# niveathika/siddhi

Measured on AMD Instinct MI355X. Metric: events/sec ingested + matches/sec (partitioned pattern, 1–8 GPU); % HBM peak, higher is better.
Workload: dtype f64; 1 GPU; P3; events_per_gpu=100000000, keys_per_gpu=10000000, micro_batch=50000896, call_size=1024, parallelism=key-sharded x1, input=prepartitioned

## Files before the change

### siddhi_amd/csrc/common.h

```cpp
#pragma once
#include <hip/hip_runtime.h>

#include <cstddef>
#include <cstdint>
#include <cstring>
#include <memory>
#include <stdexcept>
#include <string>
#include <type_traits>
#include <utility>
#include <vector>

#include "../../include/siddhi_hip.h"
#include "../../include/siddhi_ir.h"

namespace shd {

struct Error : std::runtime_error {
  int code;
  Error(int c, const std::string& m) : std::runtime_error(m), code(c) {}
};

#define SHD_HIP(call)                                                                  \
  do {                                                                                 \
// ... 145 lines not shown
};

template <class T>
__device__ __forceinline__ T gld(const T* p, int64_t i) {
  typedef __attribute__((address_space(1))) const T* GP;
  return ((GP)p)[i];
}

struct ColSet {
  const void* col[kMaxCols];
  const uint8_t* nul[kMaxCols];
  int32_t type[kMaxCols];
  int32_t ncols;
  const int64_t* ts;
  int64_t n;
};

inline int type_size(int t) {
  switch (t) {
    case SHD_T_STRING: case SHD_T_INT: case SHD_T_FLOAT: return 4;
    case SHD_T_LONG: case SHD_T_DOUBLE: return 8;
    case SHD_T_BOOL: return 1;
  }
  return 8;
}

__host__ __device__ __forceinline__ uint32_t key_bucket_mix(uint32_t k) {
  const uint32_t h = k * 0x9E3779B1u;
  return h ^ (h >> 16);
}

void scan_exclusive_u32(const uint32_t* in, uint32_t* out, int64_t n, uint32_t* total_dev,
                        DevBuf& scratch, hipStream_t s);
void radix_sort_pairs_u32(uint32_t* keys, uint32_t* vals, uint32_t* keys_alt, uint32_t* vals_alt,
                          int64_t n, int bits, DevBuf& scratch, hipStream_t s, bool& result_in_alt);
void radix_sort_pairs_u64(uint64_t* keys, uint32_t* vals, uint64_t* keys_alt, uint32_t* vals_alt,
                          int64_t n, int bits, DevBuf& scratch, hipStream_t s, bool& result_in_alt);
void radix_sort_triples_u32(uint32_t* keys, uint32_t* vals, uint32_t* w, uint32_t* keys_alt, uint32_t* vals_alt,
                            uint32_t* w_alt, int64_t n, int bits, DevBuf& scratch, hipStream_t s, bool& in_alt,
                            bool hashed = false, uint32_t kbase = 0, int shift0 = 0);
void radix_sort_triples_u64(uint64_t* keys, uint32_t* vals, uint32_t* w, uint64_t* keys_alt, uint32_t* vals_alt,
                            uint32_t* w_alt, int64_t n, int bits, DevBuf& scratch, hipStream_t s, bool& in_alt);
const uint32_t* radix_digit_totals(const DevBuf& scratch, int64_t n);
void radix_digit_scan(const uint32_t* hist, int nb, uint32_t* offs, uint32_t* dtot, hipStream_t s);
void reduce_max_u64(const uint64_t* in, int64_t n, uint64_t* out_dev, hipStream_t s);
void fill_iota_u32(uint32_t* out, int64_t n, uint32_t base, hipStream_t s);

}
```

### siddhi_amd/csrc/engine_absent.hip

```cpp
#include "engine.h"
#include "pattern_common.h"

namespace shd {

namespace {

using pat::ExtRows;
using pat::PairCtx;
using pat::BatchRowCtx;

enum : uint8_t { AS_NONE = 0, AS_FIRED = 1, AS_OPEN = 2 };

struct AbsArgs {
  ExtRows x;
  DExprSet es;
  DFilters f1, fx;
  int is_a;
  int sx;
  int64_t T;
  const int64_t* e_off;
  const int64_t* e_now;
  int ne;
};

// ... 437 lines not shown
    }
    const ExtRows x = ext(&b.cs);
    AbsArgs aa{};
    aa.x = x;
    aa.es = dset();
    aa.f1 = dfilters(f1);
    aa.fx = dfilters(fx);
    aa.is_a = isA;
    aa.sx = sx;
    aa.T = T;
    aa.e_off = d_eoff.as<int64_t>();
    aa.e_now = d_enow.as<int64_t>();
    aa.ne = ne;
    const int nblk = grid_for(n_ext, 1, 4096);
    const int64_t tile = ceil_div(ceil_div(n_ext, nblk), kBlock) * kBlock;
    const int ntile = (int)ceil_div(n_ext, tile);
    d_st.reserve(n_ext);
    d_fe.reserve(n_ext * 4);
    d_bcnt.reserve((size_t)2 * ntile * 4);
    d_boff.reserve((size_t)2 * ntile * 4);
    d_blk.reserve((size_t)ntile * sizeof(AbsOut));
    agg.reserve();
    const AbsArgs* d_aa = dev_args(aa);
    if (aa.f1.fp.ok && aa.fx.fp.ok)
      hipLaunchKernelGGL(k_abs_scan<true>, dim3(ntile), dim3(kBlock), 0, s, d_aa, n_ext, d_st.as<uint8_t>(),
                         d_fe.as<int32_t>(), d_bcnt.as<uint32_t>(), d_blk.as<AbsOut>(), tile);
    else
      hipLaunchKernelGGL(k_abs_scan<false>, dim3(ntile), dim3(kBlock), 0, s, d_aa, n_ext, d_st.as<uint8_t>(),
                         d_fe.as<int32_t>(), d_bcnt.as<uint32_t>(), d_blk.as<AbsOut>(), tile);
    SHD_CHECK_LAUNCH();
    hipLaunchKernelGGL(k_abs_fold, dim3(1), dim3(kBlock), 0, s, (const AbsOut*)d_blk.as<AbsOut>(), ntile,
                       &agg.dev()->out);
    SHD_CHECK_LAUNCH();
    scan_exclusive_u32(d_bcnt.as<uint32_t>(), d_boff.as<uint32_t>(), ntile, &agg.dev()->n_fired, d_scan, s);
    scan_exclusive_u32(d_bcnt.as<uint32_t>() + ntile, d_boff.as<uint32_t>() + ntile, ntile, &agg.dev()->n_open, d_scan,
                       s);
    agg.fetch(&AbsentTotals::out, &AbsentTotals::n_open, s);
    SHD_HIP(hipStreamSynchronize(s));
    mark("absent_scan");
    const AbsOut so = agg.host().out;
    const uint32_t n_fired = agg.host().n_fired, n_open = agg.host().n_open;
    if (so.unmono)
      throw NeedNfa("absent pattern engine: event timestamps decrease");
    d_list.reserve((size_t)std::max<uint32_t>(std::max(n_fired, n_open), 1) * 4);
    if (n_fired) {
      hipLaunchKernelGGL(k_abs_list, dim3(ntile), dim3(kBlock), 0, s, (const uint8_t*)d_st.as<uint8_t>(), n_ext, tile,
                         (uint8_t)AS_FIRED, (const uint32_t*)d_boff.as<uint32_t>(), d_list.as<uint32_t>());
      SHD_CHECK_LAUNCH();
      project(x, d_list.as<uint32_t>(), n_fired, d_fe.as<int32_t>(), d_eoff.as<int64_t>(), 0);
    }
    if (n_open) {
      hipLaunchKernelGGL(k_abs_list, dim3(ntile), dim3(kBlock), 0, s, (const uint8_t*)d_st.as<uint8_t>(), n_ext, tile,
                         (uint8_t)AS_OPEN, (const uint32_t*)d_boff.as<uint32_t>() + ntile, d_list.as<uint32_t>());
      SHD_CHECK_LAUNCH();
    }
    carry_rows(x, d_list.as<uint32_t>(), n_open, 0);
    mark("emit_carry");
    SHD_HIP(hipEventRecord(ev1, s));
    stage_end();
    SHD_HIP(hipEventSynchronize(ev1));
    float ms = 0.f;
    SHD_HIP(hipEventElapsedTime(&ms, ev0, ev1));
    seq += n;
    now = now_after;
    counters.events += n;
    counters.partials += (int64_t)so.created;
    counters.partial_scans += (int64_t)so.steps;
    counters.carry = C;
    counters.kernel_ns = (int64_t)(ms * 1e6);
// ... 110 lines not shown
```

### siddhi_amd/csrc/engine_pattern.hip

```cpp
#include <algorithm>
#include <unordered_map>
#include <cmath>
#include <cstdio>
#include <cstdlib>

#include "engine.h"
#include "knobs.h"
#include "pattern_common.h"

namespace shd {

using namespace pat;

namespace {

template <bool FAST>
__global__ __launch_bounds__(kBlock) void k_prepare(const PrepArgs* __restrict__ ap, int64_t n_ext, int64_t stride,
                                                    uint32_t* __restrict__ k32, uint64_t* __restrict__ k64,
                                                    uint32_t* __restrict__ pv, int32_t* __restrict__ tso,
                                                    PrepAgg* __restrict__ blk) {
  const PrepArgs& a = *ap;
  const DExprSet es = a.es;
  PrepAcc acc;
  const int64_t tbase = a.x.batch.ts[0];
// ... 1321 lines not shown
    if (!sts) a.dts[o] = gld(x.batch.ts, br);
    a.dseq[o] = x.seq0 + br;
  }
  a.dkey[o] = kk;
  a.dpend[o] = (uint8_t)((pend_now || (r < x.C && a.pend_old[r])) ? 1 : 0);
}

__global__ __launch_bounds__(kBlock) void k_gather_list(const GatherArgs* __restrict__ ap,
                                                        const uint32_t* __restrict__ olist, int64_t n_open,
                                                        const uint8_t* __restrict__ pst,
                                                        const uint32_t* __restrict__ spv,
                                                        const uint32_t* __restrict__ skey32,
                                                        const uint64_t* __restrict__ skey64) {
  const GatherArgs& a = *ap;
  const ExtRows& x = a.x;
  for (int64_t oi = (int64_t)blockIdx.x * kBlock + threadIdx.x; oi < n_open; oi = n_open) {
    const int64_t p = olist[oi];
    const int64_t o = oi;
    const int64_t r = pv_row(spv[p]);
    const uint64_t kk = !a.partitioned ? 0 : (a.key64 ? skey64[p] : (uint64_t)skey32[p]);
    const bool sts = a.sts32 || a.sts64;
    gather_open_row(a, o, r, kk, sts, (pst[p] & PS_PEND) != 0);
    if (sts) a.dts[o] = a.sts64 ? a.sts64[p] : gld(x.batch.ts, 0) + (int64_t)a.sts32[p];
  }
}

__global__ __launch_bounds__(kBlock) void k_gather_rec(const GatherArgs* __restrict__ ap, int64_t sub, int nsub,
                                                       const uint32_t* __restrict__ rkey,
                                                       const uint32_t* __restrict__ rpv,
                                                       const int32_t* __restrict__ rts,
                                                       const uint32_t* __restrict__ rpos,
                                                       const uint32_t* __restrict__ scnt,
                                                       const uint32_t* __restrict__ soff,
                                                       const uint8_t* __restrict__ pst) {
  const GatherArgs& a = *ap;
  const int lane = threadIdx.x & 63;
  const int st = (int)blockIdx.x * kSubPerTile + (threadIdx.x >> 6);
  const int64_t base = (int64_t)st * sub;
  const uint32_t nrec = scnt[2 * (int64_t)nsub + st];
  const int64_t tbase = gld(a.x.batch.ts, 0);
  const uint64_t below = ((uint64_t)1 << lane) - 1;
  int64_t o0 = soff[st];
  for (uint32_t i0 = 0; i0 < nrec; i0 += 64) {
    const uint32_t i = i0 + lane;
    bool valid = false, pend = false;
    if (i < nrec) {
      const uint32_t rp = rpos[base + i];
      valid = true;
      if (rp & kRecDeferred) {
        const uint8_t ps = pst[rp & ~kRecDeferred];
        valid = (ps & 0x7Fu) == PS_OPEN;
        pend = (ps & PS_PEND) != 0;
      }
    }
    const uint64_t mv = __ballot(valid);
    if (valid) {
      const int64_t o = o0 + __popcll(mv & below);
      gather_open_row(a, o, pv_row(rpv[base + i]), a.partitioned ? (uint64_t)rkey[base + i] : 0, true, pend);
      a.dts[o] = tbase + (int64_t)rts[base + i];
    }
    o0 += __popcll(mv);
  }
}

struct CarryTable {
  DevBuf col[kMaxCols], nul[kMaxCols], ts, key, seq;
  DevBuf pend;
  DevBuf half, bcol[kMaxCols], bnul[kMaxCols], bts, bseq;
  void reserve_b(int64_t n, const std::vector<int>& types) {
    n = std::max<int64_t>(n, 1);
    half.reserve(n);
    for (size_t c = 0; c < types.size(); c++) {
      bcol[c].reserve(n * type_size(types[c]));
      bnul[c].reserve(n);
    }
    bts.reserve(n * 8);
    bseq.reserve(n * 8);
  }
  ColSet colset_b(const std::vector<int>& types, int64_t n) const {
    ColSet cs{};
    cs.ncols = (int)types.size();
    for (size_t c = 0; c < types.size(); c++) {
      cs.col[c] = bcol[c].p;
      cs.nul[c] = bnul[c].as<uint8_t>();
      cs.type[c] = (int32_t)types[c];
    }
    cs.ts = bts.as<int64_t>();
    cs.n = n;
    return cs;
  }
  void reserve(int64_t n, const std::vector<int>& types) {
    for (size_t c = 0; c < types.size(); c++) {
      col[c].reserve(std::max<int64_t>(n, 1) * type_size(types[c]));
      nul[c].reserve(std::max<int64_t>(n, 1));
    }
    ts.reserve(std::max<int64_t>(n, 1) * 8);
    key.reserve(std::max<int64_t>(n, 1) * 8);
    seq.reserve(std::max<int64_t>(n, 1) * 8);
    pend.reserve(std::max<int64_t>(n, 1));
  }
  ColSet colset(const std::vector<int>& types) const {
    ColSet cs{};
    cs.ncols = (int)types.size();
    for (size_t c = 0; c < types.size(); c++) {
      cs.col[c] = col[c].p;
      cs.nul[c] = nul[c].as<uint8_t>();
      cs.type[c] = (int32_t)types[c];
    }
    cs.ts = ts.as<int64_t>();
    return cs;
  }
};

bool expr_reads_only(const Plan& p, int e, int st) {
  for (auto& in : p.exprs[e])
    if ((in.op == SHD_OP_LOAD || in.op == SHD_OP_EVNULL || in.op == SHD_OP_TS) && in.a != st) return false;
  return true;
}

int plain_load_attr(const Plan& p, int e) {
  auto& code = p.exprs[e];
  if (code.size() == 1 && code[0].op == SHD_OP_LOAD) return code[0].c & 0xFFFF;
  return -1;
}

bool find_key_equality(const Plan& p, const std::vector<int>& filters, int& attr_a, int& attr_b, int& type) {
  for (int e : filters) {
    const auto& code = p.exprs[e];
    std::vector<int> st;
    std::vector<std::pair<int, int>> kid(code.size(), {-1, -1});
    bool ok = true;
    for (int i = 0; i < (int)code.size() && ok; i++) {
// ... 632 lines not shown
                           s);
        d_dlist.reserve((size_t)n_ext * 4);
        hipLaunchKernelGGL(k_open_list, dim3(ntile), dim3(kBlock), 0, s, (const uint8_t*)d_pst.as<uint8_t>(),
                           (const uint32_t*)d_boff.as<uint32_t>(), n_ext, tile, d_dlist.as<uint32_t>(),
                           (uint32_t)PS_DEFER, 2);
        SHD_CHECK_LAUNCH();
#define SHD_LAUNCH_RLIST(FAST, TS64)                                                                               \
  hipLaunchKernelGGL((k_resume_list<false, FAST, TS64>), dim3(nlb), dim3(kBlock), 0, s, d_sa, n_ext, tile, ntile,     \
                     skey32, skey64, spv, sts32, sts64, d_match.as<int32_t>(), d_mother.as<int32_t>(),              \
                     d_pst.as<uint8_t>(), d_bcnt.as<uint32_t>(), d_blk.as<ScanOut>(), ntile,                        \
                     (const uint32_t*)d_dlist.as<uint32_t>(), (const uint32_t*)d_ndef, (const uint32_t*)nullptr, 0,  \
                     (int64_t)0, (uint32_t*)nullptr)
        if (fast2) {
          if (ts64) SHD_LAUNCH_RLIST(true, true); else SHD_LAUNCH_RLIST(true, false);
        } else {
          if (ts64) SHD_LAUNCH_RLIST(false, true); else SHD_LAUNCH_RLIST(false, false);
        }
#undef SHD_LAUNCH_RLIST
      } else if (fast2) { SHD_LAUNCH_RESUME2(false, true); }
      else { SHD_LAUNCH_RESUME2(false, false); }
    }
#undef SHD_LAUNCH_RESUME2
#undef SHD_LAUNCH_SKIP
#undef SHD_LAUNCH_RESUME_D
#undef SHD_LAUNCH_RESUME
#undef SHD_LAUNCH_SCAN
    SHD_CHECK_LAUNCH();
    hipLaunchKernelGGL(k_finish_scan, dim3(1), dim3(kBlock), 0, s, (const ScanOut*)d_blk.as<ScanOut>(),
                       rlist ? ntile + nlb : (rmode == 3 && !lockstep ? 3 : 2) * ntile,
                       d_so);
    SHD_CHECK_LAUNCH();
    mark("forward_scan");

    scan_exclusive_u32(d_bcnt.as<uint32_t>(), d_boff.as<uint32_t>(), ntile, &agg.dev()->n_match, d_scan, s);
    if (slists)
      scan_exclusive_u32(d_scnt, d_soff, nsub, &agg.dev()->n_open, d_scan, s);
    else
      scan_exclusive_u32(d_bcnt.as<uint32_t>() + ntile, d_boff.as<uint32_t>() + ntile, ntile, &agg.dev()->n_open,
                         d_scan, s);
    mark("compact");
    agg.fetch(&PatternTotals::scan, &PatternTotals::tail_, s);
    SHD_HIP(hipMemcpyAsync(&h_agg.t_last, b.cs.ts + (n - 1), 8, hipMemcpyDeviceToHost, s));
    SHD_HIP(hipStreamSynchronize(s));
    const ScanOut so = h_agg.scan;
    const uint32_t m = h_agg.n_match;
    const uint32_t n_open = h_agg.n_open;
    if (so.violation)
      throw NeedNfa("pattern engine: event timestamps decrease within a key under `within`");
    if (so.pruned) {
      have_horizon = true;
      horizon = std::max(horizon, t_end);
    }
    fin_sts32 = sts32;
    fin_sts64 = sts64;
    finish(b, x, n_ext, tile, ntile, spv, skey32, skey64, sorted64, keyed, grouped, key64, m, n_open, so, t_end,
           pg.n_cand);
  }

  void finish(const Staged& b, const ExtRows& x, int64_t n_ext, int64_t tile, int ntile, const uint32_t* spv,
              const uint32_t* skey32, const uint64_t* skey64, bool sorted64, bool keyed, bool grouped, bool key64,
              uint32_t m, uint32_t n_open, const ScanOut& so, int64_t t_end, uint64_t n_cand) {
    hipStream_t s = stream;
    const int64_t n = b.n;
    if (m > 0) {
      d_pj.reserve((int64_t)m * 4);
      d_pi.reserve((int64_t)m * 4);
      d_pj_alt.reserve((int64_t)m * 4);
      d_pi_alt.reserve((int64_t)m * 4);
      if (logical == 2) {
        d_se1.reserve((int64_t)m * 4);
        d_sot.reserve((int64_t)m * 4);
      }
      hipLaunchKernelGGL(k_emit_pairs, dim3(ntile), dim3(kBlock), 0, s, (const uint8_t*)d_pst.as<uint8_t>(),
                         (const uint32_t*)d_boff.as<uint32_t>(), (const int32_t*)d_match.as<int32_t>(), spv, n_ext,
                         tile, logical, (const int32_t*)d_mother.as<int32_t>(), d_pj.as<uint32_t>(),
                         d_pi.as<uint32_t>(), d_se1.as<uint32_t>(), d_sot.as<int32_t>());
      SHD_CHECK_LAUNCH();
      int bits = 0;
      while (bits < 32 && ((uint64_t)n_ext >> bits)) bits++;
      if (logical) bits++;
      bool in_alt = false;
      radix_sort_pairs_u32(d_pj.as<uint32_t>(), d_pi.as<uint32_t>(), d_pj_alt.as<uint32_t>(),
                           d_pi_alt.as<uint32_t>(), m, bits, d_sort, s, in_alt);
      const uint32_t* pj = in_alt ? d_pj_alt.as<uint32_t>() : d_pj.as<uint32_t>();
      const uint32_t* pi = in_alt ? d_pi_alt.as<uint32_t>() : d_pi.as<uint32_t>();
      if (!gmembers.empty()) {
        group_emit(b, x, pj, pi, m);
        mark("order_project");
      } else {
        out.ensure(m, s);
        ProjArgs pr{};
        pr.x = x;
        pr.es = dset();
        pr.nout = (int)outs.size();
        pr.fast = 1;
        for (size_t c = 0; c < outs.size(); c++) {
          pr.outs[c] = dexpr(outs[c]);
          if (!fast_atom(outs[c], pr.oat[c])) pr.fast = 0;
        }
        pr.multi = (sA == sB);
        pr.logical = logical;
        pr.s_first = s_first;
        pr.s_second = s_second;
        pr.se1 = d_se1.as<uint32_t>();
        pr.sot = d_sot.as<int32_t>();
        pr.chunk0 = chunk_seq;
        pr.row0 = out.count;
        hipLaunchKernelGGL(k_project, dim3(grid_cover(m)), dim3(kBlock), 0, s, dev_args(pr), pj, pi, (int64_t)m,
                           out.d_chunk(), out.d_type(), out.d_ts(), out.d_vals(), out.d_nulls(), out.d_seq(),
                           out.d_sidx());
        SHD_CHECK_LAUNCH();
        out.count += m;
        if (sA != sB && !logical) chunk_seq += m;
        mark("order_project");
      }
    }

    int nxt = cur ^ 1;
    carry[nxt].reserve(n_open, typesA);
    if (n_open > 0) {
      GatherArgs ga{};
      ga.x = x;
      ga.ncols = (int)typesA.size();
      ga.partitioned = keyed;
      ga.key64 = sorted64;
      for (size_t c = 0; c < typesA.size(); c++) {
        ga.types[c] = (int32_t)typesA[c];
        ga.dcol[c] = carry[nxt].col[c].p;
        ga.dnul[c] = carry[nxt].nul[c].as<uint8_t>();
      }
      ga.dts = carry[nxt].ts.as<int64_t>();
      ga.dkey = carry[nxt].key.as<uint64_t>();
      ga.dseq = carry[nxt].seq.as<int64_t>();
      carry[cur].pend.reserve(std::max<int64_t>(C, 1));
      ga.dpend = carry[nxt].pend.as<uint8_t>();
      ga.pend_old = carry[cur].pend.as<uint8_t>();
      if (logical == 2) {
        carry[nxt].reserve_b(n_open, typesB);
        ga.and_mode = 1;
        ga.match_row = d_match.as<int32_t>();
        ga.dhalf = carry[nxt].half.as<uint8_t>();
        ga.ncolsB = (int)typesB.size();
        for (size_t c = 0; c < typesB.size(); c++) {
          ga.typesB[c] = (int32_t)typesB[c];
          ga.dcolB[c] = carry[nxt].bcol[c].p;
          ga.dnulB[c] = carry[nxt].bnul[c].as<uint8_t>();
        }
        ga.dtsB = carry[nxt].bts.as<int64_t>();
        ga.dseqB = carry[nxt].bseq.as<int64_t>();
      }
      if (keyed && !grouped) {
        ga.key64 = key64;
        skey32 = d_k32.as<uint32_t>();
        skey64 = d_k64.as<uint64_t>();
      }
      if (logical != 2) {
        ga.amask = carry_mask;
        if (grouped) {
          ga.sts32 = fin_sts32;
          ga.sts64 = fin_sts64;
          ga.key_attr = (partitioned && !sorted64 && key_col[0] >= 0 &&
                         (key_type[0] == SHD_T_STRING || key_type[0] == SHD_T_INT)) ? key_col[0] : -1;
        } else {
          ga.key_attr = -1;
        }
        if (fin_rec.on) {
          hipLaunchKernelGGL(k_gather_rec, dim3(ntile), dim3(kBlock), 0, s, dev_args(ga), fin_rec.sub, fin_rec.nsub,
                             (const uint32_t*)fin_rec.key, (const uint32_t*)fin_rec.pv, (const int32_t*)fin_rec.ts,
                             (const uint32_t*)fin_rec.pos,
                             (const uint32_t*)(d_bcnt.as<uint32_t>() + 3 * ntile),
                             (const uint32_t*)(d_boff.as<uint32_t>() + 3 * ntile),
                             (const uint8_t*)d_pst.as<uint8_t>());
        } else {
          d_olist.reserve((size_t)n_open * 4);
          hipLaunchKernelGGL(k_open_list, dim3(ntile), dim3(kBlock), 0, s, (const uint8_t*)d_pst.as<uint8_t>(),
                             (const uint32_t*)d_boff.as<uint32_t>(), n_ext, tile, d_olist.as<uint32_t>(),
                             (uint32_t)PS_OPEN, 1);
          SHD_CHECK_LAUNCH();
          hipLaunchKernelGGL(k_gather_list, dim3(grid_cover((int64_t)n_open)), dim3(kBlock), 0, s, dev_args(ga),
                             (const uint32_t*)d_olist.as<uint32_t>(), (int64_t)n_open,
                             (const uint8_t*)d_pst.as<uint8_t>(), spv, skey32, skey64);
        }
      } else {
        hipLaunchKernelGGL(k_gather_carry, dim3(ntile), dim3(kBlock), 0, s, dev_args(ga),
                           (const uint8_t*)d_pst.as<uint8_t>(), (const uint32_t*)d_boff.as<uint32_t>(), spv, skey32,
                           skey64, n_ext, tile);
      }
      SHD_CHECK_LAUNCH();
      mark("carry");
    }
    SHD_HIP(hipEventRecord(ev1, s));
    stage_end();
    SHD_HIP(hipEventSynchronize(ev1));
    float ms = 0.f;
    SHD_HIP(hipEventElapsedTime(&ms, ev0, ev1));
    cur = nxt;
    C = n_open;
    if (b.stream == sB) last_b_seq = seq + n - 1;
    seq += n;
    if (b.advance_time && t_end > now) now = t_end;
    t_last = agg.host().t_last;
    counters.events += n;
    counters.matches += m;
    counters.partial_scans += (int64_t)so.steps;
    counters.carry = C;
// ... 276 lines not shown
```

### siddhi_amd/csrc/knobs.h

```cpp
#pragma once
#include <cassert>
#include <cstdlib>

namespace shd {

#define SHD_KNOBS(X)                                                                                                  \
                                                                                                     \
  X(SYNC_CHECK, "SHD_SYNC_CHECK", FLAG, PROCESS, "synchronize after every kernel launch so a fault names its launch") \
  X(NO_FAST_PRED, "SHD_NO_FAST_PRED", FLAG, PUSH, "filters run on the expression interpreter, never pre-decoded")     \
  X(FORCE_NFA, "SHD_FORCE_NFA", FLAG, LOAD, "every state plan runs on the generic NFA engine")                        \
  X(NO_LOGICAL_SCAN, "SHD_NO_LOGICAL_SCAN", FLAG, LOAD, "`every e1 -> (e2 or/and e3)` runs on the generic NFA engine") \
  X(NO_ABSENT_SCAN, "SHD_NO_ABSENT_SCAN", FLAG, LOAD, "`every e1 -> not X for t` runs on the generic NFA engine")     \
                                                                                              \
  X(NO_HASH, "SHD_NO_HASH", FLAG, PUSH, "pattern: never sort by hashed buckets")                                      \
  X(HASH_BITS, "SHD_HASH_BITS", INT, PUSH, "pattern: sort by this many hashed-bucket bits (outside 1..32: none)")     \
  X(FUSED_SORT, "SHD_FUSED_SORT", TRISTATE, PUSH, "pattern: fused prepare + first sort pass off / on at any push size") \
  X(TS64, "SHD_TS64", FLAG, PUSH, "pattern: 64-bit sorted timestamps even when 32-bit offsets fit")                   \
  X(RESUME_MODE, "SHD_RESUME_MODE", INT, PUSH, "pattern: deferred-walk mode 0..3 (ignored where the mode cannot run)") \
  X(LOCKSTEP, "SHD_LOCKSTEP", TRISTATE, PUSH, "pattern: lockstep walks off / on wherever they can run")               \
  X(NO_BPOS, "SHD_NO_BPOS", FLAG, PUSH, "pattern: never copy e2 attributes into position order (wins over SHD_BPOS)") \
  X(BPOS, "SHD_BPOS", FLAG, PUSH, "pattern: position-major e2 attributes whenever walks are dense")                   \
  X(NO_SPLIT, "SHD_NO_SPLIT", FLAG, PUSH, "pattern: f2 through eval_fpred per step, not split per comparison")        \
  X(NO_BLOCK_SKIP, "SHD_NO_BLOCK_SKIP", FLAG, PUSH, "pattern: walks never skip 64-position blocks (wins over SHD_BLOCK_SKIP)") \
  X(BLOCK_SKIP, "SHD_BLOCK_SKIP", FLAG, PUSH, "pattern: block skipping at any key density")                           \
  X(NO_RESUME_LIST, "SHD_NO_RESUME_LIST", FLAG, PUSH, "pattern: sparse deferred walks without the compacted list")    \
  X(NO_SCAN_LISTS, "SHD_NO_SCAN_LISTS", FLAG, PUSH, "pattern: open and deferred lists by the list passes, not from the scan") \
  X(NO_IMPLICIT_KEY, "SHD_NO_IMPLICIT_KEY", FLAG, LOAD, "pattern: a key equality in f2 does not partition the plan")  \
                                                                                                  \
  X(KS_GENERIC_F1, "SHD_KS_GENERIC_F1", FLAG, PUSH, "fused sort: f1 through eval_fpred per row, not pre-decoded")     \
                                                                                                  \
  X(NFA_DEBUG, "SHD_NFA_DEBUG", FLAG, LOAD, "NFA: print window-lane decisions (and phase clocks in the prof build)")  \
  X(NFA_CHUNK, "SHD_NFA_CHUNK", INT, PUSH, "NFA: window-lane chunk length in events (at least 1)")                    \
  X(NFA_HASH1_ZERO, "SHD_NFA_HASH1_ZERO", FLAG, PUSH, "NFA: zero the first window-lane state hash (forces the fallback)") \
  X(NFA_WINDOW, "SHD_NFA_WINDOW", TRISTATE, LOAD, "NFA: 0 turns window lanes off")                                    \
  X(NFA_LIST, "SHD_NFA_LIST", INT, LOAD, "NFA: pending-list capacity per key (> 0)")                                  \
  X(NFA_PARTIALS, "SHD_NFA_PARTIALS", INT, LOAD, "NFA: partial capacity per key (> 0)")                               \
  X(NFA_EVENTS, "SHD_NFA_EVENTS", INT, LOAD, "NFA: event capacity per key (> 0)")                                     \
  X(NFA_RECORDS, "SHD_NFA_RECORDS", INT, LOAD, "NFA: record capacity per key (> 0)")                                  \
  X(NFA_TIMERS, "SHD_NFA_TIMERS", INT, LOAD, "NFA: timer capacity per key (> 0)")                                     \
                                                                                               \
  X(DEBUG_ARGS, "SHD_DEBUG_ARGS", FLAG, PUSH, "filter: print k_filter's arguments and stop before the launch")        \
  X(WCHUNK, "SHD_WCHUNK", FLAG, PUSH, "windows: the chunked walk (opt-in)")                                           \
  X(NO_WCHUNK, "SHD_NO_WCHUNK", FLAG, PUSH, "windows: never the chunked walk (wins over SHD_WCHUNK)")                 \
  X(NO_CALLWIN, "SHD_NO_CALLWIN", FLAG, PUSH, "windows: never the call-window path")                                  \
  X(FOLD_LANE, "SHD_FOLD_LANE", FLAG, PUSH, "group fold: one lane per group at any segment length")                   \
// ... 53 lines not shown
```

### siddhi_amd/csrc/primitives.hip

```cpp
#include <cstdlib>

#include "common.h"
#include "radix_tile.h"

namespace shd {

constexpr int kScanItems = 4;
constexpr int kScanTile = kBlock * kScanItems;

__device__ inline uint32_t wave_incl_scan(uint32_t v) {
  int lane = threadIdx.x & 63;
#pragma unroll
  for (int o = 1; o < 64; o <<= 1) {
    uint32_t t = __shfl_up(v, o, 64);
    if (lane >= o) v += t;
  }
  return v;
}

__device__ inline uint32_t block_excl_scan(uint32_t v, uint32_t* lds4, uint32_t* total) {
  int lane = threadIdx.x & 63, w = threadIdx.x >> 6;
  uint32_t inc = wave_incl_scan(v);
  if (lane == 63) lds4[w] = inc;
  __syncthreads();
  uint32_t pre = 0, tot = 0;
#pragma unroll
  for (int i = 0; i < kBlock / 64; i++) {
    uint32_t s = lds4[i];
    if (i < w) pre += s;
    tot += s;
  }
  __syncthreads();
  *total = tot;
  return pre + inc - v;
}
// ... 38 lines not shown
    hipLaunchKernelGGL(k_scan_down, dim3(1), dim3(kBlock), 0, s, in, n, (const uint32_t*)nullptr, out, total_dev);
    SHD_CHECK_LAUNCH();
    return;
  }
  uint32_t* bsum = scratch;
  uint32_t* boff = scratch + nb;
  hipLaunchKernelGGL(k_scan_reduce, dim3((unsigned)nb), dim3(kBlock), 0, s, in, n, bsum);
  SHD_CHECK_LAUNCH();
  scan_rec(bsum, boff, nb, nullptr, scratch + 2 * nb, s);
  hipLaunchKernelGGL(k_scan_down, dim3((unsigned)nb), dim3(kBlock), 0, s, in, n, (const uint32_t*)boff, out,
                     total_dev);
  SHD_CHECK_LAUNCH();
}

static int64_t scan_need(int64_t n) {
  int64_t need = 0, m = n;
  while (m > kScanTile) {
    int64_t nb = ceil_div(m, kScanTile);
    need += 2 * nb;
    m = nb;
  }
  return need + 64;
}

static void scan_raw(const uint32_t* in, uint32_t* out, int64_t n, uint32_t* total_dev, uint32_t* scratch,
                     hipStream_t s) {
  if (n <= 0) {
    if (total_dev) SHD_HIP(hipMemsetAsync(total_dev, 0, 4, s));
    return;
  }
  scan_rec(in, out, n, total_dev, scratch, s);
}

void scan_exclusive_u32(const uint32_t* in, uint32_t* out, int64_t n, uint32_t* total_dev, DevBuf& scratch,
                        hipStream_t s) {
  scratch.reserve(scan_need(n) * sizeof(uint32_t));
  scan_raw(in, out, n, total_dev, scratch.as<uint32_t>(), s);
}


template <class K, int R, bool H>
__global__ __launch_bounds__(kRsBlock) void k_rs_hist(const K* __restrict__ keys, int64_t n, int shift,
                                                      uint32_t* __restrict__ hist, int nb, K kb) {
  __shared__ uint32_t h[kRsWaves][256];
  const int tid = threadIdx.x, lane = tid & 63, w = tid >> 6;
  for (int i = tid; i < kRsWaves * 256; i += kRsBlock) (&h[0][0])[i] = 0;
  const int tile = rs_tile_of(blockIdx.x, nb);
  const int64_t wb = (int64_t)tile * rs_tile(R) + (int64_t)w * 64 * R;
  bool done = false;
  if constexpr (sizeof(K) == 4 && R % 4 == 0) {
    if ((int64_t)(tile + 1) * rs_tile(R) <= n) {
      const uint4* kv = reinterpret_cast<const uint4*>(keys + wb);
      uint4 q[R / 4];
#pragma unroll
      for (int i = 0; i < R / 4; i++) q[i] = kv[i * 64 + lane];
      __syncthreads();
#pragma unroll
      for (int i = 0; i < R / 4; i++) {
        atomicAdd(&h[w][rs_hdigit<H>((K)q[i].x, shift, kb)], 1u);
        atomicAdd(&h[w][rs_hdigit<H>((K)q[i].y, shift, kb)], 1u);
        atomicAdd(&h[w][rs_hdigit<H>((K)q[i].z, shift, kb)], 1u);
        atomicAdd(&h[w][rs_hdigit<H>((K)q[i].w, shift, kb)], 1u);
      }
      done = true;
    }
  }
  if (!done) {
    K k[R];
#pragma unroll
    for (int r = 0; r < R; r++) {
// ... 50 lines not shown
    pre += c;
  }
  if (tid == 0) total[d] = tot;
}

template <class K, int R, bool P2, bool H>
__global__ __launch_bounds__(kRsBlock) void k_rs_scatter(const K* __restrict__ kin, const uint32_t* __restrict__ vin,
                                                         const uint32_t* __restrict__ win, K* __restrict__ kout,
                                                         uint32_t* __restrict__ vout, uint32_t* __restrict__ wout,
                                                         int64_t n, int shift, const uint32_t* __restrict__ hist,
                                                         const uint32_t* __restrict__ offs,
                                                         const uint32_t* __restrict__ dtotal, int nb, K kb) {
  const int tid = threadIdx.x, lane = tid & 63, w = tid >> 6;
  const int tile = rs_tile_of(blockIdx.x, nb);
  const int64_t t0 = (int64_t)tile * rs_tile(R);
  const int64_t wb = t0 + (int64_t)w * 64 * R;
  const uint32_t c = tid < 256 ? hist[(int64_t)tid * nb + tile] : 0u;
  const uint32_t gr = tid < 256 ? offs[(int64_t)tid * nb + tile] : 0u;
  const uint32_t dt = tid < 256 ? dtotal[tid] : 0u;
  K k[R];
  uint32_t v[R];
  uint32_t x[P2 ? R : 1];
#pragma unroll
  for (int r = 0; r < R; r++) {
    const int64_t idx = wb + r * 64 + lane;
    const int64_t li = idx < n ? idx : n - 1;
    k[r] = kin[li];
    v[r] = vin[li];
    if (P2) x[r] = win[li];
  }
  rs_scatter_tile<K, R, P2, H>(k, v, x, n, t0, wb, shift, c, gr, dt, kb, kout, vout, wout);
}

template <class K, int R, bool P2, bool H = false>
static void radix_sort_run(K* keys, uint32_t* vals, uint32_t* w, K* keys_alt, uint32_t* vals_alt, uint32_t* w_alt,
                           int64_t n, int bits, DevBuf& scratch, hipStream_t s, bool& in_alt, K kb = 0,
                           int shift0 = 0) {
  in_alt = false;
  if (n <= 1 || bits <= 0) return;
  if ((reinterpret_cast<uintptr_t>(keys) | reinterpret_cast<uintptr_t>(keys_alt)) & 15)
    throw Error(SHD_E_ARG, "radix sort: key arrays must be 16-byte aligned");
  const int nb = (int)ceil_div(n, rs_tile(R));
  const int64_t nh = (int64_t)nb * 256;
  const size_t need = (size_t)(2 * nh + 256) * sizeof(uint32_t);
  scratch.reserve(need);
  uint32_t* hist = scratch.as<uint32_t>();
  uint32_t* offs = hist + nh;
  uint32_t* dtot = offs + nh;
  K* ki = keys; uint32_t* vi = vals; uint32_t* wi = w;
  K* ko = keys_alt; uint32_t* vo = vals_alt; uint32_t* wo = w_alt;
  for (int shift = shift0; shift < bits; shift += 8) {
    hipLaunchKernelGGL((k_rs_hist<K, R, H>), dim3(nb), dim3(kRsBlock), 0, s, (const K*)ki, n, shift, hist, nb, kb);
    SHD_CHECK_LAUNCH();
    hipLaunchKernelGGL(k_rs_digit_scan, dim3(256), dim3(kRsBlock), 0, s, (const uint32_t*)hist, nb, offs, dtot);
    SHD_CHECK_LAUNCH();
    hipLaunchKernelGGL((k_rs_scatter<K, R, P2, H>), dim3(nb), dim3(kRsBlock), 0, s, (const K*)ki, (const uint32_t*)vi,
                       (const uint32_t*)wi, ko, vo, wo, n, shift, (const uint32_t*)hist, (const uint32_t*)offs,
                       (const uint32_t*)dtot, nb, kb);
    SHD_CHECK_LAUNCH();
    std::swap(ki, ko);
    std::swap(vi, vo);
    std::swap(wi, wo);
    in_alt = !in_alt;
  }
}

void radix_digit_scan(const uint32_t* hist, int nb, uint32_t* offs, uint32_t* dtot, hipStream_t s) {
  hipLaunchKernelGGL(k_rs_digit_scan, dim3(256), dim3(kRsBlock), 0, s, hist, nb, offs, dtot);
  SHD_CHECK_LAUNCH();
}

const uint32_t* radix_digit_totals(const DevBuf& scratch, int64_t n) {
  const int64_t nh = ceil_div(n, rs_tile(kRsRounds)) * 256;
  return scratch.as<uint32_t>() + 2 * nh;
}

void radix_sort_pairs_u32(uint32_t* keys, uint32_t* vals, uint32_t* keys_alt, uint32_t* vals_alt, int64_t n,
                          int bits, DevBuf& scratch, hipStream_t s, bool& in_alt) {
  radix_sort_run<uint32_t, kRsRounds, false>(keys, vals, nullptr, keys_alt, vals_alt, nullptr, n, bits, scratch, s,
                                             in_alt);
}

void radix_sort_pairs_u64(uint64_t* keys, uint32_t* vals, uint64_t* keys_alt, uint32_t* vals_alt, int64_t n,
                          int bits, DevBuf& scratch, hipStream_t s, bool& in_alt) {
// ... 52 lines not shown
```

Baseline: 24.13 billion events/s.

## Shorten small launch chains: single-block scans, fused small radix passes, early carry gather

Adds a single-block exclusive scan kernel that handles up to four small scans in one launch, replacing the recursive multi-launch scan for small inputs. Adds a fused one-launch radix pass for sorts of at most four tiles, where each block recomputes the full histogram itself. In the pattern engine, the carry gather is launched before the host sync using the capacity of the existing carry buffer, with row writes bounded by that capacity, and is skipped after the sync when the buffer was big enough. The aim is to cut kernel launch count and host-sync latency, at the cost of redundant histogram work and possibly wasted gather work when the buffer turns out too small.

```diff
diff --git a/siddhi_amd/csrc/common.h b/siddhi_amd/csrc/common.h
--- a/siddhi_amd/csrc/common.h
+++ b/siddhi_amd/csrc/common.h
@@ -201,6 +201,14 @@
 
 void scan_exclusive_u32(const uint32_t* in, uint32_t* out, int64_t n, uint32_t* total_dev,
                         DevBuf& scratch, hipStream_t s);
+struct ScanJob {
+  const uint32_t* in;
+  uint32_t* out;
+  int64_t n;
+  uint32_t* total_dev;
+};
+constexpr int kScanBatchMax = 4;
+void scan_exclusive_u32_batch(const ScanJob* jobs, int njobs, DevBuf& scratch, hipStream_t s);
 void radix_sort_pairs_u32(uint32_t* keys, uint32_t* vals, uint32_t* keys_alt, uint32_t* vals_alt,
                           int64_t n, int bits, DevBuf& scratch, hipStream_t s, bool& result_in_alt);
 void radix_sort_pairs_u64(uint64_t* keys, uint32_t* vals, uint64_t* keys_alt, uint32_t* vals_alt,
diff --git a/siddhi_amd/csrc/engine_absent.hip b/siddhi_amd/csrc/engine_absent.hip
--- a/siddhi_amd/csrc/engine_absent.hip
+++ b/siddhi_amd/csrc/engine_absent.hip
@@ -493,9 +493,10 @@
     hipLaunchKernelGGL(k_abs_fold, dim3(1), dim3(kBlock), 0, s, (const AbsOut*)d_blk.as<AbsOut>(), ntile,
                        &agg.dev()->out);
     SHD_CHECK_LAUNCH();
-    scan_exclusive_u32(d_bcnt.as<uint32_t>(), d_boff.as<uint32_t>(), ntile, &agg.dev()->n_fired, d_scan, s);
-    scan_exclusive_u32(d_bcnt.as<uint32_t>() + ntile, d_boff.as<uint32_t>() + ntile, ntile, &agg.dev()->n_open, d_scan,
-                       s);
+    const ScanJob scans[2] = {
+        {d_bcnt.as<uint32_t>(), d_boff.as<uint32_t>(), ntile, &agg.dev()->n_fired},
+        {d_bcnt.as<uint32_t>() + ntile, d_boff.as<uint32_t>() + ntile, ntile, &agg.dev()->n_open}};
+    scan_exclusive_u32_batch(scans, 2, d_scan, s);
     agg.fetch(&AbsentTotals::out, &AbsentTotals::n_open, s);
     SHD_HIP(hipStreamSynchronize(s));
     mark("absent_scan");
diff --git a/siddhi_amd/csrc/engine_pattern.hip b/siddhi_amd/csrc/engine_pattern.hip
--- a/siddhi_amd/csrc/engine_pattern.hip
+++ b/siddhi_amd/csrc/engine_pattern.hip
@@ -1377,7 +1377,7 @@
                                                        const uint32_t* __restrict__ rpos,
                                                        const uint32_t* __restrict__ scnt,
                                                        const uint32_t* __restrict__ soff,
-                                                       const uint8_t* __restrict__ pst) {
+                                                       const uint8_t* __restrict__ pst, int64_t cap_rows) {
   const GatherArgs& a = *ap;
   const int lane = threadIdx.x & 63;
   const int st = (int)blockIdx.x * kSubPerTile + (threadIdx.x >> 6);
@@ -1399,8 +1399,8 @@
       }
     }
     const uint64_t mv = __ballot(valid);
-    if (valid) {
-      const int64_t o = o0 + __popcll(mv & below);
+    const int64_t o = o0 + __popcll(mv & below);
+    if (valid && o < cap_rows) {
       gather_open_row(a, o, pv_row(rpv[base + i]), a.partitioned ? (uint64_t)rkey[base + i] : 0, true, pend);
       a.dts[o] = tbase + (int64_t)rts[base + i];
     }
@@ -1443,6 +1443,13 @@
     key.reserve(std::max<int64_t>(n, 1) * 8);
     seq.reserve(std::max<int64_t>(n, 1) * 8);
     pend.reserve(std::max<int64_t>(n, 1));
+  }
+  int64_t rows(const std::vector<int>& types) const {
+    size_t r = std::min(std::min(ts.cap, key.cap), seq.cap) / 8;
+    r = std::min(r, pend.cap);
+    for (size_t c = 0; c < types.size(); c++)
+      r = std::min(r, std::min(col[c].cap / (size_t)type_size(types[c]), nul[c].cap));
+    return (int64_t)r;
   }
   ColSet colset(const std::vector<int>& types) const {
     ColSet cs{};
@@ -2141,13 +2148,19 @@
     SHD_CHECK_LAUNCH();
     mark("forward_scan");
 
-    scan_exclusive_u32(d_bcnt.as<uint32_t>(), d_boff.as<uint32_t>(), ntile, &agg.dev()->n_match, d_scan, s);
+    ScanJob scans[2] = {{d_bcnt.as<uint32_t>(), d_boff.as<uint32_t>(), ntile, &agg.dev()->n_match},
+                        {d_bcnt.as<uint32_t>() + ntile, d_boff.as<uint32_t>() + ntile, ntile, &agg.dev()->n_open}};
     if (slists)
-      scan_exclusive_u32(d_scnt, d_soff, nsub, &agg.dev()->n_open, d_scan, s);
-    else
-      scan_exclusive_u32(d_bcnt.as<uint32_t>() + ntile, d_boff.as<uint32_t>() + ntile, ntile, &agg.dev()->n_open,
-                         d_scan, s);
+      scans[1] = ScanJob{d_scnt, d_soff, nsub, &agg.dev()->n_open};
+    scan_exclusive_u32_batch(scans, 2, d_scan, s);
     mark("compact");
+    fin_sts32 = sts32;
+    fin_sts64 = sts64;
+    int64_t early_rows = 0;
+    if (fin_rec.on && !knob_on(Knob::NO_SHORT_CHAINS)) {
+      early_rows = carry[cur ^ 1].rows(typesA);
+      if (early_rows > 0) launch_gather_rec(gather_args(x, cur ^ 1, keyed, grouped, key64, sorted64), ntile, early_rows);
+    }
     agg.fetch(&PatternTotals::scan, &PatternTotals::tail_, s);
     SHD_HIP(hipMemcpyAsync(&h_agg.t_last, b.cs.ts + (n - 1), 8, hipMemcpyDeviceToHost, s));
     SHD_HIP(hipStreamSynchronize(s));
@@ -2160,15 +2173,55 @@
       have_horizon = true;
       horizon = std::max(horizon, t_end);
     }
-    fin_sts32 = sts32;
-    fin_sts64 = sts64;
     finish(b, x, n_ext, tile, ntile, spv, skey32, skey64, sorted64, keyed, grouped, key64, m, n_open, so, t_end,
-           pg.n_cand);
+           pg.n_cand, early_rows);
+  }
+
+  GatherArgs gather_args(const ExtRows& x, int nxt, bool keyed, bool grouped, bool key64, bool sorted64) {
+    GatherArgs ga{};
+    ga.x = x;
+    ga.ncols = (int)typesA.size();
+    ga.partitioned = keyed;
+    ga.key64 = sorted64;
+    for (size_t c = 0; c < typesA.size(); c++) {
+      ga.types[c] = (int32_t)typesA[c];
+      ga.dcol[c] = carry[nxt].col[c].p;
+      ga.dnul[c] = carry[nxt].nul[c].as<uint8_t>();
+    }
+    ga.dts = carry[nxt].ts.as<int64_t>();
+    ga.dkey = carry[nxt].key.as<uint64_t>();
+    ga.dseq = carry[nxt].seq.as<int64_t>();
+    carry[cur].pend.reserve(std::max<int64_t>(C, 1));
+    ga.dpend = carry[nxt].pend.as<uint8_t>();
+    ga.pend_old = carry[cur].pend.as<uint8_t>();
+    if (keyed && !grouped) ga.key64 = key64;
+    if (logical != 2) {
+      ga.amask = carry_mask;
+      if (grouped) {
+        ga.sts32 = fin_sts32;
+        ga.sts64 = fin_sts64;
+        ga.key_attr = (partitioned && !sorted64 && key_col[0] >= 0 &&
+                       (key_type[0] == SHD_T_STRING || key_type[0] == SHD_T_INT)) ? key_col[0] : -1;
+      } else {
+        ga.key_attr = -1;
+      }
+    }
+    return ga;
+  }
+
+  void launch_gather_rec(const GatherArgs& ga, int ntile, int64_t rows) {
+    hipLaunchKernelGGL(k_gather_rec, dim3(ntile), dim3(kBlock), 0, stream, dev_args(ga), fin_rec.sub, fin_rec.nsub,
+                       (const uint32_t*)fin_rec.key, (const uint32_t*)fin_rec.pv, (const int32_t*)fin_rec.ts,
+                       (const uint32_t*)fin_rec.pos, (const uint32_t*)(d_bcnt.as<uint32_t>() + 3 * ntile),
+                       (const uint32_t*)(d_boff.as<uint32_t>() + 3 * ntile), (const uint8_t*)d_pst.as<uint8_t>(),
+                       rows);
+    SHD_CHECK_LAUNCH();
   }
 
   void finish(const Staged& b, const ExtRows& x, int64_t n_ext, int64_t tile, int ntile, const uint32_t* spv,
               const uint32_t* skey32, const uint64_t* skey64, bool sorted64, bool keyed, bool grouped, bool key64,
-              uint32_t m, uint32_t n_open, const ScanOut& so, int64_t t_end, uint64_t n_cand) {
+              uint32_t m, uint32_t n_open, const ScanOut& so, int64_t t_end, uint64_t n_cand,
+              int64_t early_rows = 0) {
     hipStream_t s = stream;
     const int64_t n = b.n;
     if (m > 0) {
@@ -2227,23 +2280,10 @@
 
     int nxt = cur ^ 1;
     carry[nxt].reserve(n_open, typesA);
-    if (n_open > 0) {
-      GatherArgs ga{};
-      ga.x = x;
-      ga.ncols = (int)typesA.size();
-      ga.partitioned = keyed;
-      ga.key64 = sorted64;
-      for (size_t c = 0; c < typesA.size(); c++) {
-        ga.types[c] = (int32_t)typesA[c];
-        ga.dcol[c] = carry[nxt].col[c].p;
-        ga.dnul[c] = carry[nxt].nul[c].as<uint8_t>();
-      }
-      ga.dts = carry[nxt].ts.as<int64_t>();
-      ga.dkey = carry[nxt].key.as<uint64_t>();
-      ga.dseq = carry[nxt].seq.as<int64_t>();
-      carry[cur].pend.reserve(std::max<int64_t>(C, 1));
-      ga.dpend = carry[nxt].pend.as<uint8_t>();
-      ga.pend_old = carry[cur].pend.as<uint8_t>();
+    if (n_open > 0 && fin_rec.on && (int64_t)n_open <= early_rows) {
+      mark("carry");
+    } else if (n_open > 0) {
+      GatherArgs ga = gather_args(x, nxt, keyed, grouped, key64, sorted64);
       if (logical == 2) {
         carry[nxt].reserve_b(n_open, typesB);
         ga.and_mode = 1;
@@ -2259,27 +2299,12 @@
         ga.dseqB = carry[nxt].bseq.as<int64_t>();
       }
       if (keyed && !grouped) {
-        ga.key64 = key64;
         skey32 = d_k32.as<uint32_t>();
         skey64 = d_k64.as<uint64_t>();
       }
       if (logical != 2) {
-        ga.amask = carry_mask;
-        if (grouped) {
-          ga.sts32 = fin_sts32;
-          ga.sts64 = fin_sts64;
-          ga.key_attr = (partitioned && !sorted64 && key_col[0] >= 0 &&
-                         (key_type[0] == SHD_T_STRING || key_type[0] == SHD_T_INT)) ? key_col[0] : -1;
-        } else {
-          ga.key_attr = -1;
-        }
         if (fin_rec.on) {
-          hipLaunchKernelGGL(k_gather_rec, dim3(ntile), dim3(kBlock), 0, s, dev_args(ga), fin_rec.sub, fin_rec.nsub,
-                             (const uint32_t*)fin_rec.key, (const uint32_t*)fin_rec.pv, (const int32_t*)fin_rec.ts,
-                             (const uint32_t*)fin_rec.pos,
-                             (const uint32_t*)(d_bcnt.as<uint32_t>() + 3 * ntile),
-                             (const uint32_t*)(d_boff.as<uint32_t>() + 3 * ntile),
-                             (const uint8_t*)d_pst.as<uint8_t>());
+          launch_gather_rec(ga, ntile, carry[nxt].rows(typesA));
         } else {
           d_olist.reserve((size_t)n_open * 4);
           hipLaunchKernelGGL(k_open_list, dim3(ntile), dim3(kBlock), 0, s, (const uint8_t*)d_pst.as<uint8_t>(),
diff --git a/siddhi_amd/csrc/knobs.h b/siddhi_amd/csrc/knobs.h
--- a/siddhi_amd/csrc/knobs.h
+++ b/siddhi_amd/csrc/knobs.h
@@ -11,6 +11,8 @@
   X(FORCE_NFA, "SHD_FORCE_NFA", FLAG, LOAD, "every state plan runs on the generic NFA engine")                        \
   X(NO_LOGICAL_SCAN, "SHD_NO_LOGICAL_SCAN", FLAG, LOAD, "`every e1 -> (e2 or/and e3)` runs on the generic NFA engine") \
   X(NO_ABSENT_SCAN, "SHD_NO_ABSENT_SCAN", FLAG, LOAD, "`every e1 -> not X for t` runs on the generic NFA engine")     \
+                                                                                                  \
+  X(NO_SHORT_CHAINS, "SHD_NO_SHORT_CHAINS", FLAG, PUSH, "test hook: recursive scans, three-launch radix passes, pattern carry gather after the sync") \
                                                                                               \
   X(NO_HASH, "SHD_NO_HASH", FLAG, PUSH, "pattern: never sort by hashed buckets")                                      \
   X(HASH_BITS, "SHD_HASH_BITS", INT, PUSH, "pattern: sort by this many hashed-bucket bits (outside 1..32: none)")     \
diff --git a/siddhi_amd/csrc/primitives.hip b/siddhi_amd/csrc/primitives.hip
--- a/siddhi_amd/csrc/primitives.hip
+++ b/siddhi_amd/csrc/primitives.hip
@@ -1,6 +1,7 @@
 #include <cstdlib>
 
 #include "common.h"
+#include "knobs.h"
 #include "radix_tile.h"
 
 namespace shd {
@@ -105,10 +106,109 @@
   scan_rec(in, out, n, total_dev, scratch, s);
 }
 
+constexpr int kScanOneBlock = 1024;
+constexpr int kScanOneItems = 16;
+constexpr int kScanOneChunk = kScanOneBlock * kScanOneItems;
+constexpr int64_t kScanOneCap = 16384;
+
+struct ScanJobs {
+  ScanJob job[kScanBatchMax];
+};
+
+__global__ __launch_bounds__(kScanOneBlock) void k_scan_one(ScanJobs jobs) {
+  __shared__ uint32_t wsum[kScanOneBlock / 64];
+  const ScanJob j = jobs.job[blockIdx.x];
+  const uint32_t* in = j.in;
+  uint32_t* out = j.out;
+  const int n = (int)j.n;
+  const int tid = threadIdx.x, lane = tid & 63, w = tid >> 6;
+  const bool vec = ((reinterpret_cast<uintptr_t>(j.in) | reinterpret_cast<uintptr_t>(j.out)) & 15) == 0;
+  uint32_t carry = 0;
+  for (int base = 0; base < n; base += kScanOneChunk) {
+    const int b = base + tid * kScanOneItems;
+    const bool full = vec && b + kScanOneItems <= n;
+    uint32_t v[kScanOneItems];
+    if (full) {
+      const uint4* p = reinterpret_cast<const uint4*>(in + b);
+#pragma unroll
+      for (int i = 0; i < kScanOneItems / 4; i++) {
+        const uint4 q = p[i];
+        v[4 * i] = q.x;
+        v[4 * i + 1] = q.y;
+        v[4 * i + 2] = q.z;
+        v[4 * i + 3] = q.w;
+      }
+    } else {
+#pragma unroll
+      for (int i = 0; i < kScanOneItems; i++) v[i] = b + i < n ? in[b + i] : 0u;
+    }
+    uint32_t sum = 0;
+#pragma unroll
+    for (int i = 0; i < kScanOneItems; i++) sum += v[i];
+    const uint32_t inc = wave_incl_scan(sum);
+    if (lane == 63) wsum[w] = inc;
+    __syncthreads();
+    uint32_t pre = carry + inc - sum, tot = 0;
+#pragma unroll
+    for (int i = 0; i < kScanOneBlock / 64; i++) {
+      const uint32_t x = wsum[i];
+      if (i < w) pre += x;
+      tot += x;
+    }
+    __syncthreads();
+    carry += tot;
+#pragma unroll
+    for (int i = 0; i < kScanOneItems; i++) {
+      const uint32_t c = v[i];
+      v[i] = pre;
+      pre += c;
+    }
+    if (full) {
+      uint4* p = reinterpret_cast<uint4*>(out + b);
+#pragma unroll
+      for (int i = 0; i < kScanOneItems / 4; i++) p[i] = make_uint4(v[4 * i], v[4 * i + 1], v[4 * i + 2], v[4 * i + 3]);
+    } else {
+#pragma unroll
+      for (int i = 0; i < kScanOneItems; i++)
+        if (b + i < n) out[b + i] = v[i];
+    }
+  }
+  if (j.total_dev && tid == 0) *j.total_dev = carry;
+}
+
+static bool short_chains() { return !knob_on(Knob::NO_SHORT_CHAINS); }
+
+static void scan_one_launch(const ScanJob* jobs, int njobs, hipStream_t s) {
+  ScanJobs a{};
+  for (int i = 0; i < njobs; i++) {
+    a.job[i] = jobs[i];
+    if (a.job[i].n < 0) a.job[i].n = 0;
+  }
+  hipLaunchKernelGGL(k_scan_one, dim3(njobs), dim3(kScanOneBlock), 0, s, a);
+  SHD_CHECK_LAUNCH();
+}
+
 void scan_exclusive_u32(const uint32_t* in, uint32_t* out, int64_t n, uint32_t* total_dev, DevBuf& scratch,
                         hipStream_t s) {
+  if (n > 0 && n <= kScanOneCap && short_chains()) {
+    const ScanJob j{in, out, n, total_dev};
+    scan_one_launch(&j, 1, s);
+    return;
+  }
   scratch.reserve(scan_need(n) * sizeof(uint32_t));
   scan_raw(in, out, n, total_dev, scratch.as<uint32_t>(), s);
+}
+
+void scan_exclusive_u32_batch(const ScanJob* jobs, int njobs, DevBuf& scratch, hipStream_t s) {
+  if (njobs < 0 || njobs > kScanBatchMax) throw Error(SHD_E_ARG, "scan batch: at most 4 jobs");
+  bool one = njobs > 0 && short_chains();
+  for (int i = 0; one && i < njobs; i++) one = jobs[i].n <= kScanOneCap;
+  if (one) {
+    scan_one_launch(jobs, njobs, s);
+    return;
+  }
+  for (int i = 0; i < njobs; i++)
+    scan_exclusive_u32(jobs[i].in, jobs[i].out, jobs[i].n, jobs[i].total_dev, scratch, s);
 }
 
 
@@ -225,10 +325,105 @@
   rs_scatter_tile<K, R, P2, H>(k, v, x, n, t0, wb, shift, c, gr, dt, kb, kout, vout, wout);
 }
 
+constexpr int kRsSmallTiles = 4;
+constexpr int kRsSmallUnroll = 8;
+
+template <class K, int R, bool P2, bool H>
+__global__ __launch_bounds__(kRsBlock) void k_rs_small(const K* __restrict__ kin, const uint32_t* __restrict__ vin,
+                                                       const uint32_t* __restrict__ win, K* __restrict__ kout,
+                                                       uint32_t* __restrict__ vout, uint32_t* __restrict__ wout,
+                                                       int n, int shift, uint32_t* __restrict__ dtotal, K kb) {
+  constexpr int T = rs_tile(R);
+  static_assert(T % 4 == 0, "a 16-byte group of 32-bit keys lies in one tile");
+  __shared__ uint32_t h[kRsWaves][3][256];
+  const int tid = threadIdx.x, lane = tid & 63, w = tid >> 6;
+  const int tile = blockIdx.x;
+  for (int i = tid; i < kRsWaves * 3 * 256; i += kRsBlock) (&h[0][0][0])[i] = 0;
+  __syncthreads();
+  uint32_t* hw = &h[w][0][0];
+  auto seg = [tile](int u) { return u < tile ? 0 : u == tile ? 256 : 512; };
+  int done = 0;
+  if constexpr (sizeof(K) == 4) {
+    const int nv = n >> 2;
+    const uint4* kv = reinterpret_cast<const uint4*>(kin);
+    constexpr int kStep = kRsBlock * kRsSmallUnroll;
+    auto load = [&](uint4 (&q)[kRsSmallUnroll], int i0) {
+#pragma unroll
+      for (int u = 0; u < kRsSmallUnroll; u++) {
+        const int i = i0 + u * kRsBlock + tid;
+        q[u] = kv[i < nv ? i : nv - 1];
+      }
+    };
+    auto count = [&](const uint4 (&q)[kRsSmallUnroll], int i0) {
+#pragma unroll
+      for (int u = 0; u < kRsSmallUnroll; u++) {
+        const int i = i0 + u * kRsBlock + tid;
+        if (i < nv) {
+          uint32_t* hs = hw + seg(i / (T / 4));
+          atomicAdd(&hs[rs_hdigit<H>((K)q[u].x, shift, kb)], 1u);
+          atomicAdd(&hs[rs_hdigit<H>((K)q[u].y, shift, kb)], 1u);
+          atomicAdd(&hs[rs_hdigit<H>((K)q[u].z, shift, kb)], 1u);
+          atomicAdd(&hs[rs_hdigit<H>((K)q[u].w, shift, kb)], 1u);
+        }
+      }
+    };
+    uint4 qa[kRsSmallUnroll], qb[kRsSmallUnroll];
+    if (nv > 0) load(qa, 0);
+    for (int i0 = 0; i0 < nv; i0 += 2 * kStep) {
+      const bool more = i0 + kStep < nv;
+      if (more) load(qb, i0 + kStep);
+      count(qa, i0);
+      if (i0 + 2 * kStep < nv) load(qa, i0 + 2 * kStep);
+      if (more) count(qb, i0 + kStep);
+    }
+    done = nv << 2;
+  }
+  for (int i0 = done; i0 < n; i0 += kRsBlock * kRsSmallUnroll) {
+    K q[kRsSmallUnroll];
+#pragma unroll
+    for (int u = 0; u < kRsSmallUnroll; u++) {
+      const int i = i0 + u * kRsBlock + tid;
+      q[u] = kin[i < n ? i : n - 1];
+    }
+#pragma unroll
+    for (int u = 0; u < kRsSmallUnroll; u++) {
+      const int i = i0 + u * kRsBlock + tid;
+      if (i < n) atomicAdd(&hw[seg(i / T) + rs_hdigit<H>(q[u], shift, kb)], 1u);
+    }
+  }
+  const int64_t t0 = (int64_t)tile * T;
+  const int64_t wb = t0 + (int64_t)w * 64 * R;
+  K k[R];
+  uint32_t v[R];
+  uint32_t x[P2 ? R : 1];
+#pragma unroll
+  for (int r = 0; r < R; r++) {
+    const int64_t idx = wb + r * 64 + lane;
+    const int64_t li = idx < n ? idx : n - 1;
+    k[r] = kin[li];
+    v[r] = vin[li];
+    if (P2) x[r] = win[li];
+  }
+  __syncthreads();
+  uint32_t c = 0, gr = 0, dt = 0;
+  if (tid < 256) {
+    uint32_t after = 0;
+#pragma unroll
+    for (int i = 0; i < kRsWaves; i++) {
+      gr += h[i][0][tid];
+      c += h[i][1][tid];
+      after += h[i][2][tid];
+    }
+    dt = gr + c + after;
+    if (tile == 0) dtotal[tid] = dt;
+  }
+  rs_scatter_tile<K, R, P2, H>(k, v, x, n, t0, wb, shift, c, gr, dt, kb, kout, vout, wout);
+}
+
 template <class K, int R, bool P2, bool H = false>
 static void radix_sort_run(K* keys, uint32_t* vals, uint32_t* w, K* keys_alt, uint32_t* vals_alt, uint32_t* w_alt,
                            int64_t n, int bits, DevBuf& scratch, hipStream_t s, bool& in_alt, K kb = 0,
-                           int shift0 = 0) {
+                           int shift0 = 0, int small = -1) {
   in_alt = false;
   if (n <= 1 || bits <= 0) return;
   if ((reinterpret_cast<uintptr_t>(keys) | reinterpret_cast<uintptr_t>(keys_alt)) & 15)
@@ -242,7 +437,18 @@
   uint32_t* dtot = offs + nh;
   K* ki = keys; uint32_t* vi = vals; uint32_t* wi = w;
   K* ko = keys_alt; uint32_t* vo = vals_alt; uint32_t* wo = w_alt;
+  const bool one = small < 0 ? nb <= kRsSmallTiles && short_chains() : small != 0;
   for (int shift = shift0; shift < bits; shift += 8) {
+    if (one) {
+      hipLaunchKernelGGL((k_rs_small<K, R, P2, H>), dim3(nb), dim3(kRsBlock), 0, s, (const K*)ki, (const uint32_t*)vi,
+                         (const uint32_t*)wi, ko, vo, wo, (int)n, shift, dtot, kb);
+      SHD_CHECK_LAUNCH();
+      std::swap(ki, ko);
+      std::swap(vi, vo);
+      std::swap(wi, wo);
+      in_alt = !in_alt;
+      continue;
+    }
     hipLaunchKernelGGL((k_rs_hist<K, R, H>), dim3(nb), dim3(kRsBlock), 0, s, (const K*)ki, n, shift, hist, nb, kb);
     SHD_CHECK_LAUNCH();
     hipLaunchKernelGGL(k_rs_digit_scan, dim3(256), dim3(kRsBlock), 0, s, (const uint32_t*)hist, nb, offs, dtot);
```

New measurement: 23.63 billion events/s. -2.1%, worse.
